# andrewmilson/sandstorm

Hardware: AMD Instinct MI355X
Metric: prove_wall_time_s (lower is better)
Workload: dtype u256 (Fp252, Montgomery R=2^256, 8 x u32 limbs)

## Files before the change

sandstorm_amd/csrc/capi.hip:

```cpp
#include <hip/hip_runtime.h>
#include <dlfcn.h>
#include <algorithm>
#include <cstdarg>
#include <chrono>
#include <cstdio>
#include <cstdlib>
#include <cstring>
#include <map>
#include <mutex>
#include <string>
#include <tuple>
#include <utility>
#include <vector>

#include "../../include/sandstorm_hip.h"
#include "fp252.h"
#include "fp252_host.h"
#include "kernels.h"
#include "quotient_gen.h"
#include "ext_scan.h"
#include "gl_ntt.h"

using namespace ss;

// ... 955 lines not shown
                          const void *d_leaves, uint64_t n, uint8_t *d_nodes, uint8_t *d_tags,
                          uint8_t root_out[33]) {
    return ss_merkle_build_ex(ctx, tree_kind, n_friendly_layers, leaf_kind, d_leaves, n, SS_ORDER_NATURAL, d_nodes, d_tags, root_out);
}
ss_status ss_merkle_build_ex(ss_ctx *ctx, int tree_kind, uint32_t n_friendly_layers, int leaf_kind,
                             const void *d_leaves, uint64_t n, int leaf_order, uint8_t *d_nodes, uint8_t *d_tags,
                             uint8_t root_out[33]) {
    if (!ctx || !d_leaves || !d_nodes) return fail(SS_ERR_INVALID, "NULL argument");
    if (n < 2 || (n & (n - 1))) return fail(SS_ERR_INVALID, "n must be a power of two >= 2");
    if (tree_kind < 0 || tree_kind > SS_TREE_SHA256) return fail(SS_ERR_INVALID, "bad tree kind");
    if (tree_kind == SS_TREE_SHA256 && leaf_kind != SS_LEAF_DIGEST) return fail(SS_ERR_UNSUPPORTED, "SHA-256 trees take digests as leaves");
    if (leaf_kind != SS_LEAF_DIGEST && leaf_kind != SS_LEAF_FELT) return fail(SS_ERR_INVALID, "bad leaf kind %d", leaf_kind);
    if (leaf_order != SS_ORDER_NATURAL && leaf_order != SS_ORDER_BITREV) return fail(SS_ERR_INVALID, "bad leaf order %d", leaf_order);
    uint32_t log_n = 0;
    while ((1ull << log_n) < n) ++log_n;
    if (leaf_kind == SS_LEAF_FELT && leaf_order == SS_ORDER_BITREV) {
        ss_status pst = ctx->ensure_scratch2(n * sizeof(Fp));
        if (pst != SS_OK) return pst;
        HIP_TRY(launch_bitrev_copy(ctx->stream, (const Fp *)d_leaves, log_n, (Fp *)ctx->scratch2));
        d_leaves = ctx->scratch2;
    }
    hipStream_t s = ctx->stream;
    const int hk = tree_kind == SS_TREE_KECCAK ? SS_HASH_KECCAK : tree_kind == SS_TREE_KECCAK_M20 ? SS_HASH_KECCAK_M20
                 : tree_kind == SS_TREE_BLAKE2S ? SS_HASH_BLAKE2S : tree_kind == SS_TREE_SHA256 ? SS_HASH_SHA256 : SS_HASH_BLAKE2S_M20;
    if (tree_kind == SS_TREE_FRIENDLY && !ctx->ped) HIP_TRY(pedersen_tables_create(s, &ctx->ped));
    Fp *ped_tmp = nullptr;
    if (tree_kind == SS_TREE_FRIENDLY) {
        ss_status st = ctx->ensure_scratch(PEDERSEN_TMP_FELTS_PER_HASH * (n / 2) * sizeof(Fp));
        if (st != SS_OK) return st;
        ped_tmp = (Fp *)ctx->scratch;
    }
    HIP_TRY(hipMemsetAsync(d_nodes, 0, 64, s));
    if (d_tags) HIP_TRY(hipMemsetAsync(d_tags, 0, 2 * n, s));
    if (leaf_kind == SS_LEAF_FELT) {
        HIP_TRY(launch_felts_to_be(s, (const Fp *)d_leaves, n, d_nodes + 32 * n));
    } else {
        HIP_TRY(hipMemcpyAsync(d_nodes + 32 * n, d_leaves, 32 * n, hipMemcpyDeviceToDevice, s));
        if (d_tags && tree_kind == SS_TREE_FRIENDLY) HIP_TRY(hipMemsetAsync(d_tags + n, 1, n, s));
    }
    ss_ctx::Scope prof(ctx, SS_PROF_MERKLE);
    for (uint32_t d = log_n; d-- > 0;) {
        const uint64_t count = 1ull << d;
        const uint8_t *in = d_nodes + 32 * (2 * count);
        uint8_t *out = d_nodes + 32 * count;
        const bool leaf_level = d == log_n - 1;
        if (tree_kind == SS_TREE_FRIENDLY) {
            const bool pedersen = leaf_kind == SS_LEAF_FELT || d < n_friendly_layers;
            if (leaf_level && leaf_kind == SS_LEAF_FELT) {
                HIP_TRY(launch_pedersen_felt_pairs(s, ctx->ped, (const Fp *)d_leaves, count, out, ped_tmp));
            } else if (pedersen) {
                HIP_TRY(launch_pedersen_pairs(s, ctx->ped, in, count, out, ped_tmp));
            } else {
                HIP_TRY(launch_hash_pairs(s, SS_HASH_BLAKE2S_M20, in, count, out));
                if (d_tags) HIP_TRY(hipMemsetAsync(d_tags + count, 1, count, s));
            }
        } else if (leaf_level && leaf_kind == SS_LEAF_FELT) {
            HIP_TRY(launch_hash_felt_pairs(s, hk, (const Fp *)d_leaves, count, out));
        } else {
            HIP_TRY(launch_hash_pairs(s, hk, in, count, out));
        }
    }
    if (root_out) {
        HIP_TRY(hipMemcpyAsync(root_out, d_nodes + 32, 32, hipMemcpyDeviceToHost, s));
        root_out[32] = 0;
        if (d_tags) HIP_TRY(hipMemcpyAsync(root_out + 32, d_tags + 1, 1, hipMemcpyDeviceToHost, s));
        HIP_TRY(hipStreamSynchronize(s));
        if (!d_tags && tree_kind == SS_TREE_FRIENDLY)
            root_out[32] = (leaf_kind == SS_LEAF_FELT || n_friendly_layers > 0) ? 0 : 1;
    }
    return SS_OK;
}

// ... 1743 lines not shown
```

sandstorm_amd/csrc/deep.hip:

```cpp
#include <hip/hip_runtime.h>
#include <cstdlib>
#include "fp252.h"
#include "fl252.h"
#include "inv252.h"
#include "kernels.h"

namespace ss {

__device__ __forceinline__ Fp dload(const Fp *p) {
    const uint4 *q = reinterpret_cast<const uint4 *>(p);
    uint4 a = q[0], b = q[1];
    Fp r;
    r.v[0] = a.x; r.v[1] = a.y; r.v[2] = a.z; r.v[3] = a.w;
    r.v[4] = b.x; r.v[5] = b.y; r.v[6] = b.z; r.v[7] = b.w;
    return r;
}
__device__ __forceinline__ void dstore(Fp *p, const Fp &x) {
    uint4 *q = reinterpret_cast<uint4 *>(p);
    q[0] = make_uint4(x.v[0], x.v[1], x.v[2], x.v[3]);
    q[1] = make_uint4(x.v[4], x.v[5], x.v[6], x.v[7]);
}

struct ReduceArgs {
    const Fp *in[MAX_COLS];
// ... 149 lines not shown
    const uint64_t out_len = in_len >> levels;
    uint32_t gx = (uint32_t)((out_len + 127) / 128);
    if (gx > 16384) gx = 16384;
    if (gx == 0) gx = 1;
    const dim3 grid(gx, narrays), block(128);
    const int cn = canonical ? 1 : 0;
    const size_t lds = (size_t)max_points * (36u << levels);
    if (lds > 64 * 1024) return hipErrorInvalidValue;
    if (levels == 4) hipLaunchKernelGGL(ood_fold_kernel<4>, grid, block, lds, st, d_arrays, d_points, out_len, cn);
    else if (levels == 3) hipLaunchKernelGGL(ood_fold_kernel<3>, grid, block, lds, st, d_arrays, d_points, out_len, cn);
    else if (levels == 2) hipLaunchKernelGGL(ood_fold_kernel<2>, grid, block, lds, st, d_arrays, d_points, out_len, cn);
    else hipLaunchKernelGGL(ood_fold_kernel<1>, grid, block, lds, st, d_arrays, d_points, out_len, cn);
    return hipGetLastError();
}

__global__ __launch_bounds__(128) void batch_inverse_kernel(Fp *__restrict__ D, uint64_t nchunks, uint32_t log_chunk,
                                                            Fp offset, Fp w, Fp step, Fp step_inv, Fp z, int r280) {
    const uint64_t c = blockIdx.x * (uint64_t)blockDim.x + threadIdx.x;
    if (c >= nchunks) return;
    const uint64_t CH = 1ull << log_chunk;
    const Fl sl = fl_from_fp(step), sil = fl_from_fp(step_inv), zl = fl_from_fp(z);
    Fl x = fl_from_fp(fp_mul(offset, fp_pow_u64(w, c)));
    Fl run = fl_one();
    for (uint64_t k = 0; k < CH; ++k) {
        dstore(D + c + k * nchunks, fl_pack(run));
        run = fl_mul(fl_sub_c<2, 1>(x, zl), run);
        x = fl_mul(x, sl);
    }
    Fl inv = fl_from_fp(fp_inv_safegcd(fl_to_fp(fl_weak_reduce(run))));
    if (r280) { Fp two24 = fp_zero(); two24.v[0] = 1u << 24; inv = fl_mul(inv, fl_from_fp(fp_to_mont(two24))); }
    for (uint64_t k = CH; k-- > 0;) {
        x = fl_mul(x, sil);
        const Fl pre = fl_from_fp(dload(D + c + k * nchunks));
        dstore(D + c + k * nchunks, fl_to_fp(fl_mul(inv, pre)));
        inv = fl_mul(fl_sub_c<2, 1>(x, zl), inv);
    }
}

static uint32_t batch_inverse_log_chunk(uint32_t log_N) {
    uint32_t log_chunk = log_N > 17 ? log_N - 17 : 0;
    if (log_chunk < 4) log_chunk = log_N < 4 ? log_N : 4;
    if (log_chunk > 7) log_chunk = 7;
    static const char *env = getenv("SS_BATCH_INV_LOG_CHUNK");
    if (env) { const uint32_t v = (uint32_t)atoi(env); if (v >= 1 && v <= 10 && v <= log_N) log_chunk = v; }
    return log_chunk;
}

hipError_t launch_batch_inverse(hipStream_t st, Fp *D, uint32_t log_N, const Fp &offset, const Fp &w,
                                const Fp &w_inv, const Fp &z, bool r280) {
    const uint32_t log_chunk = batch_inverse_log_chunk(log_N);
    const uint64_t nchunks = 1ull << (log_N - log_chunk);
    hipLaunchKernelGGL(batch_inverse_kernel, dim3((uint32_t)((nchunks + 127) / 128)), dim3(128), 0, st, D, nchunks,
                       log_chunk, offset, w, fp_pow_u64(w, nchunks), fp_pow_u64(w_inv, nchunks), z, r280 ? 1 : 0);
    return hipGetLastError();
}

hipError_t launch_batch_inverse_range(hipStream_t st, Fp *D, uint64_t len, const Fp &x0, const Fp &w, const Fp &w_inv,
                                      const Fp &z, bool r280) {
    const uint32_t log_chunk = BATCH_INVERSE_RANGE_LOG_CHUNK;
    const uint64_t nchunks = len >> log_chunk;
    if (nchunks == 0) return hipSuccess;
    hipLaunchKernelGGL(batch_inverse_kernel, dim3((uint32_t)((nchunks + 127) / 128)), dim3(128), 0, st, D, nchunks,
                       log_chunk, x0, w, fp_pow_u64(w, nchunks), fp_pow_u64(w_inv, nchunks), z, r280 ? 1 : 0);
    return hipGetLastError();
}

struct DeepArgs {
    const Fp *trace[MAX_COLS];
    const Fp *comp[4];
    const Fp *D;
    const Fp *Dc;
    const uint32_t *tap_shift;
    const Fp *tap_coef;
    const uint32_t *col_desc;
    const Fp *comp_coef;
    Fp comp_k;
    uint32_t ncoldesc, ncomp, log_stride;
    uint64_t count;
    uint32_t d_bias, d_mask;
// ... 201 lines not shown
```

sandstorm_amd/csrc/hash.hip:

```cpp
#include <hip/hip_runtime.h>
#include <cstring>
#include "fp252.h"
#include "kernels.h"

namespace ss {

__constant__ uint64_t KECCAK_RC[24] = {
    0x0000000000000001ull, 0x0000000000008082ull, 0x800000000000808aull, 0x8000000080008000ull,
    0x000000000000808bull, 0x0000000080000001ull, 0x8000000080008081ull, 0x8000000000008009ull,
    0x000000000000008aull, 0x0000000000000088ull, 0x0000000080008009ull, 0x000000008000000aull,
    0x000000008000808bull, 0x800000000000008bull, 0x8000000000008089ull, 0x8000000000008003ull,
    0x8000000000008002ull, 0x8000000000000080ull, 0x000000000000800aull, 0x800000008000000aull,
    0x8000000080008081ull, 0x8000000000008080ull, 0x0000000080000001ull, 0x8000000080008008ull};

struct K64 { uint32_t lo, hi; };
__device__ __forceinline__ K64 k_split(uint64_t x) { K64 r; r.lo = (uint32_t)x; r.hi = (uint32_t)(x >> 32); return r; }
__device__ __forceinline__ uint64_t k_join(const K64 &x) { return ((uint64_t)x.hi << 32) | x.lo; }
template <int N>
__device__ __forceinline__ K64 k_rotl(const K64 &x) {
    K64 r;
    if (N == 0) { r = x; }
    else if (N == 32) { r.lo = x.hi; r.hi = x.lo; }
    else if (N < 32) {
        r.hi = __builtin_amdgcn_alignbit(x.hi, x.lo, 32 - N);
// ... 2 lines not shown
        r.hi = __builtin_amdgcn_alignbit(x.lo, x.hi, 64 - N);
        r.lo = __builtin_amdgcn_alignbit(x.hi, x.lo, 64 - N);
    }
    return r;
}
__device__ __forceinline__ uint32_t k_xor3(uint32_t a, uint32_t b, uint32_t c) { return __builtin_amdgcn_bitop3_b32(a, b, c, 0x96); }
__device__ __forceinline__ uint32_t k_chi(uint32_t a, uint32_t b, uint32_t c) { return __builtin_amdgcn_bitop3_b32(a, b, c, 0xD2); }
__device__ __forceinline__ K64 k_xor5(const K64 &a, const K64 &b, const K64 &c, const K64 &d, const K64 &e) {
    K64 r; r.lo = k_xor3(k_xor3(a.lo, b.lo, c.lo), d.lo, e.lo); r.hi = k_xor3(k_xor3(a.hi, b.hi, c.hi), d.hi, e.hi); return r;
}
__device__ __forceinline__ K64 k_xor(const K64 &a, const K64 &b) { K64 r; r.lo = a.lo ^ b.lo; r.hi = a.hi ^ b.hi; return r; }
__device__ __forceinline__ K64 k_chi64(const K64 &a, const K64 &b, const K64 &c) { K64 r; r.lo = k_chi(a.lo, b.lo, c.lo); r.hi = k_chi(a.hi, b.hi, c.hi); return r; }
template <int N>
__device__ __forceinline__ K64 k_xrot(const K64 &a, const K64 &d) { return k_rotl<N>(k_xor(a, d)); }

__device__ __forceinline__ void keccak_f1600(uint64_t st[25]) {
    K64 s[25];
#pragma unroll
    for (int i = 0; i < 25; ++i) s[i] = k_split(st[i]);
#pragma unroll 1
    for (int round = 0; round < 24; ++round) {
        const K64 c0 = k_xor5(s[0], s[5], s[10], s[15], s[20]), c1 = k_xor5(s[1], s[6], s[11], s[16], s[21]);
        const K64 c2 = k_xor5(s[2], s[7], s[12], s[17], s[22]), c3 = k_xor5(s[3], s[8], s[13], s[18], s[23]);
        const K64 c4 = k_xor5(s[4], s[9], s[14], s[19], s[24]);
        const K64 d0 = k_xor(c4, k_rotl<1>(c1)), d1 = k_xor(c0, k_rotl<1>(c2)), d2 = k_xor(c1, k_rotl<1>(c3));
        const K64 d3 = k_xor(c2, k_rotl<1>(c4)), d4 = k_xor(c3, k_rotl<1>(c0));
        const K64 b0 = k_xor(s[0], d0);
        const K64 b10 = k_xrot<1>(s[1], d1), b20 = k_xrot<62>(s[2], d2), b5 = k_xrot<28>(s[3], d3);
        const K64 b15 = k_xrot<27>(s[4], d4), b16 = k_xrot<36>(s[5], d0), b1 = k_xrot<44>(s[6], d1);
        const K64 b11 = k_xrot<6>(s[7], d2), b21 = k_xrot<55>(s[8], d3), b6 = k_xrot<20>(s[9], d4);
        const K64 b7 = k_xrot<3>(s[10], d0), b17 = k_xrot<10>(s[11], d1), b2 = k_xrot<43>(s[12], d2);
        const K64 b12 = k_xrot<25>(s[13], d3), b22 = k_xrot<39>(s[14], d4), b23 = k_xrot<41>(s[15], d0);
        const K64 b8 = k_xrot<45>(s[16], d1), b18 = k_xrot<15>(s[17], d2), b3 = k_xrot<21>(s[18], d3);
        const K64 b13 = k_xrot<8>(s[19], d4), b14 = k_xrot<18>(s[20], d0), b24 = k_xrot<2>(s[21], d1);
        const K64 b9 = k_xrot<61>(s[22], d2), b19 = k_xrot<56>(s[23], d3), b4 = k_xrot<14>(s[24], d4);
        s[0] = k_chi64(b0, b1, b2); s[1] = k_chi64(b1, b2, b3); s[2] = k_chi64(b2, b3, b4); s[3] = k_chi64(b3, b4, b0); s[4] = k_chi64(b4, b0, b1);
        s[5] = k_chi64(b5, b6, b7); s[6] = k_chi64(b6, b7, b8); s[7] = k_chi64(b7, b8, b9); s[8] = k_chi64(b8, b9, b5); s[9] = k_chi64(b9, b5, b6);
        s[10] = k_chi64(b10, b11, b12); s[11] = k_chi64(b11, b12, b13); s[12] = k_chi64(b12, b13, b14); s[13] = k_chi64(b13, b14, b10); s[14] = k_chi64(b14, b10, b11);
        s[15] = k_chi64(b15, b16, b17); s[16] = k_chi64(b16, b17, b18); s[17] = k_chi64(b17, b18, b19); s[18] = k_chi64(b18, b19, b15); s[19] = k_chi64(b19, b15, b16);
        s[20] = k_chi64(b20, b21, b22); s[21] = k_chi64(b21, b22, b23); s[22] = k_chi64(b22, b23, b24); s[23] = k_chi64(b23, b24, b20); s[24] = k_chi64(b24, b20, b21);
        const uint64_t rc = KECCAK_RC[round];
        s[0].lo ^= (uint32_t)rc; s[0].hi ^= (uint32_t)(rc >> 32);
    }
#pragma unroll
    for (int i = 0; i < 25; ++i) st[i] = k_join(s[i]);
}

__device__ __forceinline__ uint32_t bswap32(uint32_t x) { return __builtin_bswap32(x); }
__device__ __forceinline__ uint64_t bswap64(uint64_t x) { return __builtin_bswap64(x); }

__device__ __forceinline__ uint64_t felt_msg_lane(const uint64_t *elem, int k) {
    return bswap64(elem[3 - k]);
}

__device__ __forceinline__ void keccak_store_digest(const uint64_t s[25], uint8_t *out, bool mask20) {
    uint64_t o2 = s[2], o3 = s[3];
    if (mask20) { o2 &= 0xffffffffull; o3 = 0; }
    ulonglong2 *q = reinterpret_cast<ulonglong2 *>(out);
    q[0] = make_ulonglong2(s[0], s[1]);
    q[1] = make_ulonglong2(o2, o3);
}

template <typename Fetch>
__device__ __forceinline__ void keccak_absorb_felts(uint64_t s[25], uint32_t nelem, Fetch fetch) {
    const uint32_t data_lanes = 4 * nelem;
    const uint32_t nblocks = data_lanes / 17 + 1;
    for (uint32_t blk = 0; blk < nblocks; ++blk) {
#pragma unroll
        for (int pos = 0; pos < 17; ++pos) {
            const uint32_t lane = blk * 17 + pos;
            if (lane < data_lanes) s[pos] ^= felt_msg_lane(fetch(lane >> 2), lane & 3);
            else if (lane == data_lanes) s[pos] ^= 0x01ull;
        }
        if (blk == nblocks - 1) s[16] ^= 0x8000000000000000ull;
        keccak_f1600(s);
    }
}

__device__ __forceinline__ uint64_t digest_slot(uint64_t row, uint32_t brev_bits) {
    return brev_bits ? (__brevll(row) >> (64u - brev_bits)) : row;
}

__global__ __launch_bounds__(256) void keccak_rows_kernel(ConstColPtrs cols, uint32_t ncols, uint64_t nrows,
                                                          uint8_t *__restrict__ out, int mask20, uint32_t brev_bits) {
    for (uint64_t row = blockIdx.x * (uint64_t)blockDim.x + threadIdx.x; row < nrows;
         row += (uint64_t)gridDim.x * blockDim.x) {
        uint64_t s[25];
#pragma unroll
        for (int i = 0; i < 25; ++i) s[i] = 0;
        keccak_absorb_felts(s, ncols, [&](uint32_t c) {
            return reinterpret_cast<const uint64_t *>(cols.p[c]) + 4 * row;
        });
        keccak_store_digest(s, out + 32 * digest_slot(row, brev_bits), mask20 != 0);
    }
}

__global__ __launch_bounds__(256) void keccak_rows_u64_kernel(ConstColPtrs segs, uint32_t nseg, uint32_t seg_len, uint64_t nrows,
                                                              uint8_t *__restrict__ out) {
    const uint32_t data_lanes = nseg * seg_len, nblocks = data_lanes / 17 + 1;
    for (uint64_t row = blockIdx.x * (uint64_t)blockDim.x + threadIdx.x; row < nrows; row += (uint64_t)gridDim.x * blockDim.x) {
        uint64_t s[25];
#pragma unroll
        for (int i = 0; i < 25; ++i) s[i] = 0;
        uint32_t seg = 0, e = 0;
        for (uint32_t blk = 0; blk < nblocks; ++blk) {
#pragma unroll
            for (int pos = 0; pos < 17; ++pos) {
// ... 8 lines not shown
            }
            if (blk == nblocks - 1) s[16] ^= 0x8000000000000000ull;
            keccak_f1600(s);
        }
        keccak_store_digest(s, out + 32 * row, false);
    }
}
__global__ void gather_rows_u64_kernel(ConstColPtrs segs, uint32_t nseg, uint32_t seg_len, const uint64_t *__restrict__ idx, uint32_t nidx,
                                       uint64_t *__restrict__ out) {
    const uint32_t per = nseg * seg_len, t = blockIdx.x * blockDim.x + threadIdx.x;
    if (t >= nidx * per) return;
    const uint32_t j = t / per, r = t - j * per, s = r / seg_len, e = r - s * seg_len;
    out[t] = reinterpret_cast<const uint64_t *>(segs.p[s])[idx[j] * seg_len + e];
}

__global__ __launch_bounds__(256) void keccak_felt_pairs_kernel(const uint64_t *__restrict__ felts, uint64_t count,
                                                                uint8_t *__restrict__ out, int mask20) {
    for (uint64_t k = blockIdx.x * (uint64_t)blockDim.x + threadIdx.x; k < count;
         k += (uint64_t)gridDim.x * blockDim.x) {
        uint64_t s[25];
#pragma unroll
        for (int i = 0; i < 25; ++i) s[i] = 0;
        keccak_absorb_felts(s, 2, [&](uint32_t c) { return felts + 4 * (2 * k + c); });
        keccak_store_digest(s, out + 32 * k, mask20 != 0);
    }
}

__global__ __launch_bounds__(256) void keccak_pairs_kernel(const uint8_t *__restrict__ in, uint64_t count,
                                                           uint8_t *__restrict__ out, int mask20) {
    for (uint64_t k = blockIdx.x * (uint64_t)blockDim.x + threadIdx.x; k < count;
         k += (uint64_t)gridDim.x * blockDim.x) {
        uint64_t s[25];
        const ulonglong2 *q = reinterpret_cast<const ulonglong2 *>(in + 64 * k);
#pragma unroll
        for (int i = 0; i < 4; ++i) { ulonglong2 v = q[i]; s[2 * i] = v.x; s[2 * i + 1] = v.y; }
        s[8] = 0x01ull;
#pragma unroll
        for (int i = 9; i < 25; ++i) s[i] = 0;
        s[16] = 0x8000000000000000ull;
        keccak_f1600(s);
        keccak_store_digest(s, out + 32 * k, mask20 != 0);
    }
}

__device__ __forceinline__ uint32_t rotr32(uint32_t x, int n) { return __builtin_rotateright32(x, n); }

#define B2S_G(a, b, c, d, x, y)                       \
    a = a + b + (x); d = rotr32(d ^ a, 16);           \
    c = c + d;       b = rotr32(b ^ c, 12);           \
    a = a + b + (y); d = rotr32(d ^ a, 8);            \
    c = c + d;       b = rotr32(b ^ c, 7);

#define B2S_ROUND(s0, s1, s2, s3, s4, s5, s6, s7, s8, s9, s10, s11, s12, s13, s14, s15) \
    B2S_G(v0, v4, v8, v12, m[s0], m[s1]);   B2S_G(v1, v5, v9, v13, m[s2], m[s3]);       \
    B2S_G(v2, v6, v10, v14, m[s4], m[s5]);  B2S_G(v3, v7, v11, v15, m[s6], m[s7]);      \
// ... 62 lines not shown
    }
}

__global__ __launch_bounds__(256) void blake2s_rows_kernel(ConstColPtrs cols, uint32_t ncols, uint64_t nrows,
                                                           uint8_t *__restrict__ out, int mask20, uint32_t brev_bits) {
    for (uint64_t row = blockIdx.x * (uint64_t)blockDim.x + threadIdx.x; row < nrows;
         row += (uint64_t)gridDim.x * blockDim.x) {
        uint32_t h[8];
        blake2s_hash_felts(h, ncols, [&](uint32_t c) {
            return load_fp(reinterpret_cast<const uint8_t *>(cols.p[c]) + 32 * row);
        });
        blake2s_store_digest(h, out + 32 * digest_slot(row, brev_bits), mask20 != 0);
    }
}

__global__ __launch_bounds__(256) void blake2s_felt_pairs_kernel(const Fp *__restrict__ felts, uint64_t count,
                                                                 uint8_t *__restrict__ out, int mask20) {
    for (uint64_t k = blockIdx.x * (uint64_t)blockDim.x + threadIdx.x; k < count;
         k += (uint64_t)gridDim.x * blockDim.x) {
        uint32_t h[8];
        blake2s_hash_felts(h, 2, [&](uint32_t c) { return load_fp(felts + 2 * k + c); });
        blake2s_store_digest(h, out + 32 * k, mask20 != 0);
    }
}

__global__ __launch_bounds__(256) void blake2s_pairs_kernel(const uint8_t *__restrict__ in, uint64_t count,
                                                            uint8_t *__restrict__ out, int mask20) {
    for (uint64_t k = blockIdx.x * (uint64_t)blockDim.x + threadIdx.x; k < count;
         k += (uint64_t)gridDim.x * blockDim.x) {
        uint32_t h[8], m[16];
        const uint4 *q = reinterpret_cast<const uint4 *>(in + 64 * k);
#pragma unroll
        for (int i = 0; i < 4; ++i) { uint4 v = q[i]; m[4 * i] = v.x; m[4 * i + 1] = v.y; m[4 * i + 2] = v.z; m[4 * i + 3] = v.w; }
        blake2s_init(h);
        blake2s_compress(h, m, 64, true);
        blake2s_store_digest(h, out + 32 * k, mask20 != 0);
    }
}

__global__ __launch_bounds__(256) void felts_to_be_kernel(const Fp *__restrict__ felts, uint64_t count,
                                                          uint8_t *__restrict__ out) {
    for (uint64_t k = blockIdx.x * (uint64_t)blockDim.x + threadIdx.x; k < count;
         k += (uint64_t)gridDim.x * blockDim.x) {
        Fp e = load_fp(felts + k);
        uint4 *q = reinterpret_cast<uint4 *>(out + 32 * k);
        q[0] = make_uint4(bswap32(e.v[7]), bswap32(e.v[6]), bswap32(e.v[5]), bswap32(e.v[4]));
        q[1] = make_uint4(bswap32(e.v[3]), bswap32(e.v[2]), bswap32(e.v[1]), bswap32(e.v[0]));
    }
}

struct Digest32 { uint64_t w[4]; };

__global__ void pow_prefix_kernel(int coin_kind, Digest32 digest, uint32_t bits, uint64_t *__restrict__ prefix) {
    if (threadIdx.x != 0 || blockIdx.x != 0) return;
    const uint64_t magic = 0x0123456789ABCDEDull;
    if (coin_kind == 0) {
        uint64_t s[25];
#pragma unroll
        for (int k = 0; k < 25; ++k) s[k] = 0;
        s[0] = bswap64(magic);
        s[1] = digest.w[0]; s[2] = digest.w[1]; s[3] = digest.w[2]; s[4] = digest.w[3];
        s[5] = (uint64_t)(bits & 0xffu) | (0x01ull << 8);
        s[16] = 0x8000000000000000ull;
// ... 190 lines not shown
    if (kind == 0) hipLaunchKernelGGL(keccak_rows_u64_kernel, dim3(grid_for(nrows, 256, 1u << 20)), dim3(256), 0, st, segs, nseg, seg_len, nrows, digests);
    else if (kind == 2) hipLaunchKernelGGL(sha256_rows_u64_kernel, dim3(grid_for(nrows, 256, 1u << 20)), dim3(256), 0, st, segs, nseg, seg_len, nrows, digests);
    else hipLaunchKernelGGL(blake2s_rows_u64_kernel, dim3(grid_for(nrows, 256, 1u << 20)), dim3(256), 0, st, segs, nseg, seg_len, nrows, digests);
    return hipGetLastError();
}
hipError_t launch_gather_rows_u64(hipStream_t st, const ConstColPtrs &segs, uint32_t nseg, uint32_t seg_len, const uint64_t *d_idx, uint32_t nidx,
                                  uint64_t *d_out) {
    const uint32_t total = nidx * nseg * seg_len;
    if (!total) return hipSuccess;
    hipLaunchKernelGGL(gather_rows_u64_kernel, dim3((total + 255) / 256), dim3(256), 0, st, segs, nseg, seg_len, d_idx, nidx, d_out);
    return hipGetLastError();
}
hipError_t launch_hash_rows(hipStream_t st, int kind, const ConstColPtrs &cols, uint32_t ncols,
                            uint64_t nrows, uint32_t brev_bits, uint8_t *digests) {
    const uint32_t grid = grid_for(nrows, 256, 1u << 20);
    if (kind == 0 || kind == 1)
        hipLaunchKernelGGL(keccak_rows_kernel, dim3(grid), dim3(256), 0, st, cols, ncols, nrows, digests, kind == 1, brev_bits);
    else
        hipLaunchKernelGGL(blake2s_rows_kernel, dim3(grid), dim3(256), 0, st, cols, ncols, nrows, digests, kind == 3, brev_bits);
    return hipGetLastError();
}
__global__ __launch_bounds__(256) void bitrev_copy_kernel(const Fp *__restrict__ src, uint32_t log_n, Fp *__restrict__ dst) {
    const uint64_t n = 1ull << log_n;
    for (uint64_t i = blockIdx.x * (uint64_t)blockDim.x + threadIdx.x; i < n; i += (uint64_t)gridDim.x * blockDim.x) {
        const uint64_t j = log_n ? (__brevll(i) >> (64u - log_n)) : 0;
        const uint4 *q = reinterpret_cast<const uint4 *>(src + j);
        uint4 *d = reinterpret_cast<uint4 *>(dst + i);
        d[0] = q[0]; d[1] = q[1];
    }
}
hipError_t launch_bitrev_copy(hipStream_t st, const Fp *src, uint32_t log_n, Fp *dst) {
    hipLaunchKernelGGL(bitrev_copy_kernel, dim3(grid_for(1ull << log_n, 256, 1u << 20)), dim3(256), 0, st, src, log_n, dst);
    return hipGetLastError();
}
hipError_t launch_hash_pairs(hipStream_t st, int kind, const uint8_t *in, uint64_t count, uint8_t *out) {
    const uint32_t grid = grid_for(count, 256, 1u << 20);
    if (kind == 4)
        hipLaunchKernelGGL(sha256_pairs_kernel, dim3(grid), dim3(256), 0, st, in, count, out);
    else if (kind == 0 || kind == 1)
        hipLaunchKernelGGL(keccak_pairs_kernel, dim3(grid), dim3(256), 0, st, in, count, out, kind == 1);
    else
        hipLaunchKernelGGL(blake2s_pairs_kernel, dim3(grid), dim3(256), 0, st, in, count, out, kind == 3);
    return hipGetLastError();
}
hipError_t launch_hash_felt_pairs(hipStream_t st, int kind, const Fp *felts, uint64_t count, uint8_t *out) {
    const uint32_t grid = grid_for(count, 256, 1u << 20);
    if (kind == 0 || kind == 1)
        hipLaunchKernelGGL(keccak_felt_pairs_kernel, dim3(grid), dim3(256), 0, st,
                           reinterpret_cast<const uint64_t *>(felts), count, out, kind == 1);
    else
        hipLaunchKernelGGL(blake2s_felt_pairs_kernel, dim3(grid), dim3(256), 0, st, felts, count, out, kind == 3);
    return hipGetLastError();
}
hipError_t launch_felts_to_be(hipStream_t st, const Fp *felts, uint64_t count, uint8_t *out) {
    hipLaunchKernelGGL(felts_to_be_kernel, dim3(grid_for(count, 256, 1u << 20)), dim3(256), 0, st, felts, count, out);
    return hipGetLastError();
}
hipError_t launch_pow_prefix(hipStream_t st, int coin_kind, const uint8_t digest[32], uint32_t bits,
                             uint64_t *d_prefix) {
    Digest32 d;
    memcpy(d.w, digest, 32);
    hipLaunchKernelGGL(pow_prefix_kernel, dim3(1), dim3(64), 0, st, coin_kind, d, bits, d_prefix);
    return hipGetLastError();
}
hipError_t launch_pow_grind(hipStream_t st, int coin_kind, const uint64_t *d_prefix, uint32_t bits,
                            uint64_t start, uint64_t count, unsigned long long *d_best) {
// ... 25 lines not shown
```

sandstorm_amd/csrc/kernels.h:

```cpp
#pragma once
#include <hip/hip_runtime.h>
#include <stdint.h>
#include "fp252.h"

namespace ss {

static constexpr int MAX_COLS = 16;

struct ColPtrs {
    const void *src[MAX_COLS];
    void *dst[MAX_COLS];
};
struct ConstColPtrs {
    const void *p[MAX_COLS];
};

int ntt_log_tile_max();
static constexpr size_t NTT_PLAN_ENTRY_BYTES = 36;
enum { NTT_MODE_DIT = 0, NTT_MODE_DIF = 1, NTT_MODE_CTI = 2 };
struct NttWindow { uint32_t first, log_len; };
hipError_t launch_ntt_pass(hipStream_t st, int mode, const ColPtrs &cols, uint32_t ncols, const Fp *tw,
                           uint32_t log_n, uint32_t s0, uint32_t r, uint32_t log_tile, uint32_t u_first,
                           uint32_t log_expand, uint32_t scale_pow2, bool final_pass, bool cti_trivial = true,
                           const NttWindow *win = nullptr, uint64_t tw_entries = 0);
hipError_t launch_twiddles(hipStream_t st, Fp *tw, const Fp *pow_lo, const Fp *pow_hi, const Fp *hpow,
                           uint32_t log_n, bool h_is_one, bool bitrev_levels, const NttWindow *win = nullptr, uint32_t win_stages = 0);
static inline uint64_t ntt_window_plan_entries(const NttWindow &win, uint32_t stages) { return (((uint64_t)1 << stages) - 1ull) << win.log_len; }
hipError_t launch_bitrev(hipStream_t st, Fp *a, uint32_t log_n);
hipError_t launch_mul_bench(hipStream_t st, const Fp *a, const Fp *b, Fp *out, uint64_t n, uint32_t reps);
hipError_t ntt_set_func_attributes();

hipError_t launch_hash_rows(hipStream_t st, int kind, const ConstColPtrs &cols, uint32_t ncols,
                            uint64_t nrows, uint32_t brev_bits, uint8_t *digests);
hipError_t launch_bitrev_copy(hipStream_t st, const Fp *src, uint32_t log_n, Fp *dst);
hipError_t launch_hash_pairs(hipStream_t st, int kind, const uint8_t *in, uint64_t count, uint8_t *out);
hipError_t launch_hash_felt_pairs(hipStream_t st, int kind, const Fp *felts, uint64_t count, uint8_t *out);
hipError_t launch_felts_to_be(hipStream_t st, const Fp *felts, uint64_t count, uint8_t *out);
hipError_t launch_pow_prefix(hipStream_t st, int coin_kind, const uint8_t digest[32], uint32_t bits,
                             uint64_t *d_prefix);
hipError_t launch_pow_grind(hipStream_t st, int coin_kind, const uint64_t *d_prefix, uint32_t bits,
                            uint64_t start, uint64_t count, unsigned long long *d_best);
hipError_t launch_gather32(hipStream_t st, const uint8_t *in, const uint64_t *d_idx, uint64_t n, uint8_t *out);
hipError_t launch_gather32_cols(hipStream_t st, const void *const *d_cols, uint32_t ncols, uint32_t c0, uint32_t row_cols, const uint64_t *d_idx,
                                uint64_t nidx, uint8_t *out);
hipError_t launch_gather8(hipStream_t st, const uint8_t *in, const uint64_t *d_idx, uint64_t n, uint8_t *out);

struct PedersenTables;
hipError_t pedersen_tables_create(hipStream_t st, PedersenTables **out);
void pedersen_tables_destroy(PedersenTables *t);
void pedersen_tables_trim();
static constexpr uint64_t PEDERSEN_TMP_FELTS_PER_HASH = 4;
// ... 170 lines not shown
```

Measured before the change: 0.2198.

## Add descent batch inverse, fused bitrev felt-pair hashing, specialized Keccak rows and squeeze

Batch inversion gains a recursive descent scheme that inverts a smaller squared domain and expands it four ways per level. It also adds a zero-aware fallback pass, gated by a device flag, for when a denominator vanishes. Merkle leaf hashing for felt leaves now reads bit-reversed input directly and writes big-endian leaves inside the hash kernel, which removes the separate bitrev copy and felts_to_be passes. Keccak gets column-count-specialized row kernels and a truncated final round that computes only the four output lanes. These changes add extra kernel launches and a global flag ring, and enlarge the set of template instantiations.

```diff
diff --git a/sandstorm_amd/csrc/capi.hip b/sandstorm_amd/csrc/capi.hip
--- a/sandstorm_amd/csrc/capi.hip
+++ b/sandstorm_amd/csrc/capi.hip
@@ -993,7 +993,8 @@
     if (leaf_order != SS_ORDER_NATURAL && leaf_order != SS_ORDER_BITREV) return fail(SS_ERR_INVALID, "bad leaf order %d", leaf_order);
     uint32_t log_n = 0;
     while ((1ull << log_n) < n) ++log_n;
-    if (leaf_kind == SS_LEAF_FELT && leaf_order == SS_ORDER_BITREV) {
+    const bool leaves_bitrev = leaf_kind == SS_LEAF_FELT && leaf_order == SS_ORDER_BITREV && tree_kind != SS_TREE_FRIENDLY;
+    if (leaf_kind == SS_LEAF_FELT && leaf_order == SS_ORDER_BITREV && !leaves_bitrev) {
         ss_status pst = ctx->ensure_scratch2(n * sizeof(Fp));
         if (pst != SS_OK) return pst;
         HIP_TRY(launch_bitrev_copy(ctx->stream, (const Fp *)d_leaves, log_n, (Fp *)ctx->scratch2));
@@ -1012,7 +1013,7 @@
     HIP_TRY(hipMemsetAsync(d_nodes, 0, 64, s));
     if (d_tags) HIP_TRY(hipMemsetAsync(d_tags, 0, 2 * n, s));
     if (leaf_kind == SS_LEAF_FELT) {
-        HIP_TRY(launch_felts_to_be(s, (const Fp *)d_leaves, n, d_nodes + 32 * n));
+        if (tree_kind == SS_TREE_FRIENDLY) HIP_TRY(launch_felts_to_be(s, (const Fp *)d_leaves, n, d_nodes + 32 * n));
     } else {
         HIP_TRY(hipMemcpyAsync(d_nodes + 32 * n, d_leaves, 32 * n, hipMemcpyDeviceToDevice, s));
         if (d_tags && tree_kind == SS_TREE_FRIENDLY) HIP_TRY(hipMemsetAsync(d_tags + n, 1, n, s));
@@ -1034,7 +1035,7 @@
                 if (d_tags) HIP_TRY(hipMemsetAsync(d_tags + count, 1, count, s));
             }
         } else if (leaf_level && leaf_kind == SS_LEAF_FELT) {
-            HIP_TRY(launch_hash_felt_pairs(s, hk, (const Fp *)d_leaves, count, out));
+            HIP_TRY(launch_hash_felt_pairs(s, hk, (const Fp *)d_leaves, count, leaves_bitrev, out, d_nodes + 32 * n));
         } else {
             HIP_TRY(launch_hash_pairs(s, hk, in, count, out));
         }
diff --git a/sandstorm_amd/csrc/deep.hip b/sandstorm_amd/csrc/deep.hip
--- a/sandstorm_amd/csrc/deep.hip
+++ b/sandstorm_amd/csrc/deep.hip
@@ -1,5 +1,7 @@
 #include <hip/hip_runtime.h>
+#include <atomic>
 #include <cstdlib>
+#include <mutex>
 #include "fp252.h"
 #include "fl252.h"
 #include "inv252.h"
@@ -187,26 +189,36 @@
     return hipGetLastError();
 }
 
+template <bool ZERO_AWARE>
 __global__ __launch_bounds__(128) void batch_inverse_kernel(Fp *__restrict__ D, uint64_t nchunks, uint32_t log_chunk,
-                                                            Fp offset, Fp w, Fp step, Fp step_inv, Fp z, int r280) {
+                                                            Fp offset, Fp w, Fp step, Fp step_inv, Fp z, int r280,
+                                                            uint32_t *__restrict__ flag, uint32_t ticket) {
     const uint64_t c = blockIdx.x * (uint64_t)blockDim.x + threadIdx.x;
     if (c >= nchunks) return;
+    if (ZERO_AWARE && *flag != ticket) return;
     const uint64_t CH = 1ull << log_chunk;
     const Fl sl = fl_from_fp(step), sil = fl_from_fp(step_inv), zl = fl_from_fp(z);
     Fl x = fl_from_fp(fp_mul(offset, fp_pow_u64(w, c)));
     Fl run = fl_one();
     for (uint64_t k = 0; k < CH; ++k) {
         dstore(D + c + k * nchunks, fl_pack(run));
-        run = fl_mul(fl_sub_c<2, 1>(x, zl), run);
+        Fl d = fl_sub_c<2, 1>(x, zl);
+        if (ZERO_AWARE) { d = fl_weak_reduce(d); if (fn_is_zero(d)) d = fl_one(); }
+        run = fl_mul(d, run);
         x = fl_mul(x, sl);
     }
-    Fl inv = fl_from_fp(fp_inv_safegcd(fl_to_fp(fl_weak_reduce(run))));
+    const Fp inv_fp = fp_inv_safegcd(fl_to_fp(fl_weak_reduce(run)));
+    if (!ZERO_AWARE && flag && fp_is_zero(inv_fp)) *flag = ticket;
+    Fl inv = fl_from_fp(inv_fp);
     if (r280) { Fp two24 = fp_zero(); two24.v[0] = 1u << 24; inv = fl_mul(inv, fl_from_fp(fp_to_mont(two24))); }
     for (uint64_t k = CH; k-- > 0;) {
         x = fl_mul(x, sil);
         const Fl pre = fl_from_fp(dload(D + c + k * nchunks));
-        dstore(D + c + k * nchunks, fl_to_fp(fl_mul(inv, pre)));
-        inv = fl_mul(fl_sub_c<2, 1>(x, zl), inv);
+        Fl d = fl_sub_c<2, 1>(x, zl);
+        bool zero = false;
+        if (ZERO_AWARE) { d = fl_weak_reduce(d); zero = fn_is_zero(d); if (zero) d = fl_one(); }
+        dstore(D + c + k * nchunks, zero ? fp_zero() : fl_to_fp(fl_mul(inv, pre)));
+        inv = fl_mul(d, inv);
     }
 }
 
@@ -219,13 +231,103 @@
     return log_chunk;
 }
 
+static hipError_t launch_batch_inverse_strided(hipStream_t st, Fp *D, uint64_t nchunks, uint32_t log_chunk, const Fp &x0, const Fp &w, const Fp &w_inv,
+                                               const Fp &z, bool r280, uint32_t *flag, uint32_t ticket, bool zero_aware) {
+    const dim3 grid((uint32_t)((nchunks + 127) / 128)), block(128);
+    const Fp step = fp_pow_u64(w, nchunks), step_inv = fp_pow_u64(w_inv, nchunks);
+    if (zero_aware) hipLaunchKernelGGL(batch_inverse_kernel<true>, grid, block, 0, st, D, nchunks, log_chunk, x0, w, step, step_inv, z, r280 ? 1 : 0, flag, ticket);
+    else hipLaunchKernelGGL(batch_inverse_kernel<false>, grid, block, 0, st, D, nchunks, log_chunk, x0, w, step, step_inv, z, r280 ? 1 : 0, flag, ticket);
+    return hipGetLastError();
+}
+static hipError_t launch_batch_inverse_chunks(hipStream_t st, Fp *D, uint32_t log_N, const Fp &offset, const Fp &w, const Fp &w_inv,
+                                              const Fp &z, bool r280, uint32_t *flag, uint32_t ticket, bool zero_aware) {
+    return launch_batch_inverse_strided(st, D, 1ull << (log_N - batch_inverse_log_chunk(log_N)), batch_inverse_log_chunk(log_N), offset, w, w_inv, z,
+                                        r280, flag, ticket, zero_aware);
+}
+
+__global__ __launch_bounds__(128) void inverse_descent_kernel(Fp *__restrict__ D, uint64_t q, uint64_t lanes, Fp a, Fp g, Fp step, Fp t, Fp c,
+                                                              Fp c2, int final, const uint32_t *__restrict__ flag, uint32_t ticket) {
+    const uint64_t l = blockIdx.x * (uint64_t)blockDim.x + threadIdx.x;
+    if (l >= lanes || *flag == ticket) return;
+    const Fl sl = fl_from_fp(step), tl = fl_from_fp(t), cl = fl_from_fp(c), c2l = fl_from_fp(c2);
+    Fl y = fl_from_fp(a), gp = fl_from_fp(g);
+    for (uint64_t b = l; b; b >>= 1) {
+        if (b & 1) y = fl_mul(y, gp);
+        gp = fl_sqr(gp);
+    }
+    Fp e_next = dload(D + l);
+    for (uint64_t i = l; i < q; i += lanes) {
+        const Fl e = fl_from_fp(e_next);
+        if (i + lanes < q) e_next = dload(D + i + lanes);
+        const Fl y2 = fl_sqr(y), ty = fl_mul(y, tl);
+        const Fl f0 = fl_mul(fl_add(y2, c2l), e), f1 = fl_mul(fl_sub_c<2, 1>(c2l, y2), e);
+        const Fl r0 = fl_mul(fl_add(y, cl), f0), r2 = fl_mul(fl_sub_c<2, 1>(cl, y), f0);
+        const Fl r1 = fl_mul(fl_add(ty, cl), f1), r3 = fl_mul(fl_sub_c<2, 1>(cl, ty), f1);
+        if (final) {
+            dstore(D + i, fl_to_fp(r0)); dstore(D + i + q, fl_to_fp(r1)); dstore(D + i + 2 * q, fl_to_fp(r2)); dstore(D + i + 3 * q, fl_to_fp(r3));
+        } else {
+            dstore(D + i, fl_pack(r0)); dstore(D + i + q, fl_pack(r1)); dstore(D + i + 2 * q, fl_pack(r2)); dstore(D + i + 3 * q, fl_pack(r3));
+        }
+        y = fl_mul(y, sl);
+    }
+}
+
+static constexpr uint32_t BATCH_INVERSE_DESCENT_LAST_LOG = 19, BATCH_INVERSE_DESCENT_LANES = 3 * 64 * 1024;
+static uint32_t batch_inverse_descent_last_log() {
+    if (const char *e = getenv("SS_BATCH_INV_DESCENT_LAST_LOG")) { const uint32_t v = (uint32_t)atoi(e); if (v >= 4 && v <= 40) return v; }
+    return BATCH_INVERSE_DESCENT_LAST_LOG;
+}
+
+static constexpr uint32_t DESCENT_FLAG_SLOTS = 1024, DESCENT_MAX_DEVICES = 64;
+static hipError_t descent_flag(uint32_t **flag, uint32_t *ticket) {
+    static std::mutex mu;
+    static uint32_t *ring[DESCENT_MAX_DEVICES] = {};
+    static std::atomic<uint32_t> next{0};
+    int dev = 0;
+    hipError_t e = hipGetDevice(&dev);
+    if (e != hipSuccess) return e;
+    if (dev < 0 || dev >= (int)DESCENT_MAX_DEVICES) return hipErrorInvalidDevice;
+    {
+        std::lock_guard<std::mutex> lock(mu);
+        if (!ring[dev]) {
+            uint32_t *p = nullptr;
+            if ((e = hipMalloc((void **)&p, DESCENT_FLAG_SLOTS * sizeof(uint32_t))) != hipSuccess) return e;
+            static const uint32_t zeros[DESCENT_FLAG_SLOTS] = {};
+            if ((e = hipMemcpy(p, zeros, sizeof zeros, hipMemcpyHostToDevice)) != hipSuccess) { (void)hipFree(p); return e; }
+            ring[dev] = p;
+        }
+    }
+    uint32_t k = next.fetch_add(1u) + 1u;
+    if (k == 0) k = next.fetch_add(1u) + 1u;
+    *ticket = k;
+    *flag = ring[dev] + k % DESCENT_FLAG_SLOTS;
+    return hipSuccess;
+}
+
 hipError_t launch_batch_inverse(hipStream_t st, Fp *D, uint32_t log_N, const Fp &offset, const Fp &w,
                                 const Fp &w_inv, const Fp &z, bool r280) {
-    const uint32_t log_chunk = batch_inverse_log_chunk(log_N);
-    const uint64_t nchunks = 1ull << (log_N - log_chunk);
-    hipLaunchKernelGGL(batch_inverse_kernel, dim3((uint32_t)((nchunks + 127) / 128)), dim3(128), 0, st, D, nchunks,
-                       log_chunk, offset, w, fp_pow_u64(w, nchunks), fp_pow_u64(w_inv, nchunks), z, r280 ? 1 : 0);
-    return hipGetLastError();
+    uint32_t *flag = nullptr, ticket = 0;
+    hipError_t e = descent_flag(&flag, &ticket);
+    if (e != hipSuccess) return e;
+    const uint32_t last_log = batch_inverse_descent_last_log();
+    if (log_N < last_log + 3) {
+        if ((e = launch_batch_inverse_chunks(st, D, log_N, offset, w, w_inv, z, r280, flag, ticket, false)) != hipSuccess) return e;
+        return launch_batch_inverse_chunks(st, D, log_N, offset, w, w_inv, z, r280, flag, ticket, true);
+    }
+    const uint32_t J = (log_N - last_log) & ~1u;
+    Fp a[64], g[64], gi[64], c[64];
+    a[0] = offset; g[0] = w; gi[0] = w_inv; c[0] = z;
+    for (uint32_t j = 1; j <= J; ++j) { a[j] = fp_sqr(a[j - 1]); g[j] = fp_sqr(g[j - 1]); gi[j] = fp_sqr(gi[j - 1]); c[j] = fp_sqr(c[j - 1]); }
+    if ((e = launch_batch_inverse_chunks(st, D, log_N - J, a[J], g[J], gi[J], c[J], r280, flag, ticket, false)) != hipSuccess) return e;
+    for (uint32_t j = J; j >= 2; j -= 2) {
+        const uint32_t lv = j - 2;
+        const uint64_t q = 1ull << (log_N - j);
+        const uint64_t lanes = q < BATCH_INVERSE_DESCENT_LANES ? q : BATCH_INVERSE_DESCENT_LANES;
+        hipLaunchKernelGGL(inverse_descent_kernel, dim3((uint32_t)((lanes + 127) / 128)), dim3(128), 0, st, D, q, lanes, a[lv], g[lv],
+                           fp_pow_u64(g[lv], lanes), fp_pow_u64(g[lv], q), c[lv], c[lv + 1], lv == 0 ? 1 : 0, flag, ticket);
+        if ((e = hipGetLastError()) != hipSuccess) return e;
+    }
+    return launch_batch_inverse_chunks(st, D, log_N, offset, w, w_inv, z, r280, flag, ticket, true);
 }
 
 hipError_t launch_batch_inverse_range(hipStream_t st, Fp *D, uint64_t len, const Fp &x0, const Fp &w, const Fp &w_inv,
@@ -233,9 +335,11 @@
     const uint32_t log_chunk = BATCH_INVERSE_RANGE_LOG_CHUNK;
     const uint64_t nchunks = len >> log_chunk;
     if (nchunks == 0) return hipSuccess;
-    hipLaunchKernelGGL(batch_inverse_kernel, dim3((uint32_t)((nchunks + 127) / 128)), dim3(128), 0, st, D, nchunks,
-                       log_chunk, x0, w, fp_pow_u64(w, nchunks), fp_pow_u64(w_inv, nchunks), z, r280 ? 1 : 0);
-    return hipGetLastError();
+    uint32_t *flag = nullptr, ticket = 0;
+    hipError_t e = descent_flag(&flag, &ticket);
+    if (e != hipSuccess) return e;
+    if ((e = launch_batch_inverse_strided(st, D, nchunks, log_chunk, x0, w, w_inv, z, r280, flag, ticket, false)) != hipSuccess) return e;
+    return launch_batch_inverse_strided(st, D, nchunks, log_chunk, x0, w, w_inv, z, r280, flag, ticket, true);
 }
 
 struct DeepArgs {
diff --git a/sandstorm_amd/csrc/hash.hip b/sandstorm_amd/csrc/hash.hip
--- a/sandstorm_amd/csrc/hash.hip
+++ b/sandstorm_amd/csrc/hash.hip
@@ -40,17 +40,17 @@
 template <int N>
 __device__ __forceinline__ K64 k_xrot(const K64 &a, const K64 &d) { return k_rotl<N>(k_xor(a, d)); }
 
-__device__ __forceinline__ void keccak_f1600(uint64_t st[25]) {
-    K64 s[25];
-#pragma unroll
-    for (int i = 0; i < 25; ++i) s[i] = k_split(st[i]);
+#define KECCAK_THETA(s)                                                                                                 \
+    const K64 c0 = k_xor5(s[0], s[5], s[10], s[15], s[20]), c1 = k_xor5(s[1], s[6], s[11], s[16], s[21]);               \
+    const K64 c2 = k_xor5(s[2], s[7], s[12], s[17], s[22]), c3 = k_xor5(s[3], s[8], s[13], s[18], s[23]);               \
+    const K64 c4 = k_xor5(s[4], s[9], s[14], s[19], s[24]);                                                             \
+    const K64 d0 = k_xor(c4, k_rotl<1>(c1)), d1 = k_xor(c0, k_rotl<1>(c2)), d2 = k_xor(c1, k_rotl<1>(c3));              \
+    const K64 d3 = k_xor(c2, k_rotl<1>(c4)), d4 = k_xor(c3, k_rotl<1>(c0));
+
+__device__ __forceinline__ void keccak_rounds(K64 (&s)[25], int nrounds) {
 #pragma unroll 1
-    for (int round = 0; round < 24; ++round) {
-        const K64 c0 = k_xor5(s[0], s[5], s[10], s[15], s[20]), c1 = k_xor5(s[1], s[6], s[11], s[16], s[21]);
-        const K64 c2 = k_xor5(s[2], s[7], s[12], s[17], s[22]), c3 = k_xor5(s[3], s[8], s[13], s[18], s[23]);
-        const K64 c4 = k_xor5(s[4], s[9], s[14], s[19], s[24]);
-        const K64 d0 = k_xor(c4, k_rotl<1>(c1)), d1 = k_xor(c0, k_rotl<1>(c2)), d2 = k_xor(c1, k_rotl<1>(c3));
-        const K64 d3 = k_xor(c2, k_rotl<1>(c4)), d4 = k_xor(c3, k_rotl<1>(c0));
+    for (int round = 0; round < nrounds; ++round) {
+        KECCAK_THETA(s)
         const K64 b0 = k_xor(s[0], d0);
         const K64 b10 = k_xrot<1>(s[1], d1), b20 = k_xrot<62>(s[2], d2), b5 = k_xrot<28>(s[3], d3);
         const K64 b15 = k_xrot<27>(s[4], d4), b16 = k_xrot<36>(s[5], d0), b1 = k_xrot<44>(s[6], d1);
@@ -68,8 +68,32 @@
         const uint64_t rc = KECCAK_RC[round];
         s[0].lo ^= (uint32_t)rc; s[0].hi ^= (uint32_t)(rc >> 32);
     }
+}
+
+__device__ __forceinline__ void keccak_f1600(uint64_t st[25]) {
+    K64 s[25];
+#pragma unroll
+    for (int i = 0; i < 25; ++i) s[i] = k_split(st[i]);
+    keccak_rounds(s, 24);
 #pragma unroll
     for (int i = 0; i < 25; ++i) st[i] = k_join(s[i]);
+}
+
+__device__ __forceinline__ void keccak_f1600_squeeze4(uint64_t st[25]) {
+    K64 s[25];
+#pragma unroll
+    for (int i = 0; i < 25; ++i) s[i] = k_split(st[i]);
+    keccak_rounds(s, 23);
+    {
+        KECCAK_THETA(s)
+        const K64 b0 = k_xor(s[0], d0), b1 = k_xrot<44>(s[6], d1), b2 = k_xrot<43>(s[12], d2);
+        const K64 b3 = k_xrot<21>(s[18], d3), b4 = k_xrot<14>(s[24], d4);
+        s[0] = k_chi64(b0, b1, b2); s[1] = k_chi64(b1, b2, b3); s[2] = k_chi64(b2, b3, b4); s[3] = k_chi64(b3, b4, b0);
+        const uint64_t rc = 0x8000000080008008ull;
+        s[0].lo ^= (uint32_t)rc; s[0].hi ^= (uint32_t)(rc >> 32);
+    }
+#pragma unroll
+    for (int i = 0; i < 4; ++i) st[i] = k_join(s[i]);
 }
 
 __device__ __forceinline__ uint32_t bswap32(uint32_t x) { return __builtin_bswap32(x); }
@@ -91,16 +115,64 @@
 __device__ __forceinline__ void keccak_absorb_felts(uint64_t s[25], uint32_t nelem, Fetch fetch) {
     const uint32_t data_lanes = 4 * nelem;
     const uint32_t nblocks = data_lanes / 17 + 1;
-    for (uint32_t blk = 0; blk < nblocks; ++blk) {
+    auto absorb = [&](uint32_t blk) {
 #pragma unroll
         for (int pos = 0; pos < 17; ++pos) {
             const uint32_t lane = blk * 17 + pos;
             if (lane < data_lanes) s[pos] ^= felt_msg_lane(fetch(lane >> 2), lane & 3);
             else if (lane == data_lanes) s[pos] ^= 0x01ull;
         }
-        if (blk == nblocks - 1) s[16] ^= 0x8000000000000000ull;
+    };
+    for (uint32_t blk = 0; blk + 1 < nblocks; ++blk) {
+        absorb(blk);
         keccak_f1600(s);
     }
+    absorb(nblocks - 1);
+    s[16] ^= 0x8000000000000000ull;
+    keccak_f1600_squeeze4(s);
+}
+
+template <int NC, int BLK>
+__device__ __forceinline__ void keccak_absorb_block(uint64_t s[25], const uint64_t (&m)[4 * NC]) {
+    constexpr int DL = 4 * NC, NB = DL / 17 + 1;
+    if constexpr (BLK < NB) {
+#pragma unroll
+        for (int pos = 0; pos < 17; ++pos) {
+            constexpr int base = BLK * 17;
+            if (base + pos < DL) s[pos] ^= m[base + pos < DL ? base + pos : 0];
+            else if (base + pos == DL) s[pos] ^= 0x01ull;
+        }
+        if constexpr (BLK == NB - 1) {
+            s[16] ^= 0x8000000000000000ull;
+            keccak_f1600_squeeze4(s);
+        } else {
+            keccak_f1600(s);
+        }
+        keccak_absorb_block<NC, BLK + 1>(s, m);
+    }
+}
+template <int NC>
+__device__ __forceinline__ void keccak_load_felts(uint64_t (&m)[4 * NC], const uint4 *const (&e)[NC]) {
+#pragma unroll
+    for (int c = 0; c < NC; ++c) {
+        const uint4 a = e[c][0], b = e[c][1];
+        m[4 * c + 0] = bswap64(((uint64_t)b.w << 32) | b.z);
+        m[4 * c + 1] = bswap64(((uint64_t)b.y << 32) | b.x);
+        m[4 * c + 2] = bswap64(((uint64_t)a.w << 32) | a.z);
+        m[4 * c + 3] = bswap64(((uint64_t)a.y << 32) | a.x);
+    }
+}
+template <int NC>
+__device__ __forceinline__ void keccak_hash_lanes(uint64_t s[25], const uint64_t (&m)[4 * NC]) {
+#pragma unroll
+    for (int i = 0; i < 25; ++i) s[i] = 0;
+    keccak_absorb_block<NC, 0>(s, m);
+}
+template <int NC>
+__device__ __forceinline__ void keccak_hash_felts(uint64_t s[25], const uint4 *const (&e)[NC]) {
+    uint64_t m[4 * NC];
+    keccak_load_felts<NC>(m, e);
+    keccak_hash_lanes<NC>(s, m);
 }
 
 __device__ __forceinline__ uint64_t digest_slot(uint64_t row, uint32_t brev_bits) {
@@ -117,6 +189,23 @@
         keccak_absorb_felts(s, ncols, [&](uint32_t c) {
             return reinterpret_cast<const uint64_t *>(cols.p[c]) + 4 * row;
         });
+        keccak_store_digest(s, out + 32 * digest_slot(row, brev_bits), mask20 != 0);
+    }
+}
+
+template <int NC>
+__global__ __launch_bounds__(256) void keccak_rows_w_kernel(ConstColPtrs cols, uint64_t nrows, uint8_t *__restrict__ out, int mask20,
+                                                            uint32_t brev_bits) {
+    const uint4 *col[NC];
+#pragma unroll
+    for (int c = 0; c < NC; ++c) col[c] = reinterpret_cast<const uint4 *>(cols.p[c]);
+    for (uint64_t row = blockIdx.x * (uint64_t)blockDim.x + threadIdx.x; row < nrows;
+         row += (uint64_t)gridDim.x * blockDim.x) {
+        const uint4 *e[NC];
+#pragma unroll
+        for (int c = 0; c < NC; ++c) e[c] = col[c] + 2 * row;
+        uint64_t s[25];
+        keccak_hash_felts<NC>(s, e);
         keccak_store_digest(s, out + 32 * digest_slot(row, brev_bits), mask20 != 0);
     }
 }
@@ -155,15 +244,21 @@
     out[t] = reinterpret_cast<const uint64_t *>(segs.p[s])[idx[j] * seg_len + e];
 }
 
-__global__ __launch_bounds__(256) void keccak_felt_pairs_kernel(const uint64_t *__restrict__ felts, uint64_t count,
-                                                                uint8_t *__restrict__ out, int mask20) {
+__global__ __launch_bounds__(256) void keccak_felt_pairs_kernel(const uint4 *__restrict__ felts, uint64_t count, uint8_t *__restrict__ out,
+                                                                uint8_t *__restrict__ leaves, int mask20, uint32_t brev_bits) {
     for (uint64_t k = blockIdx.x * (uint64_t)blockDim.x + threadIdx.x; k < count;
          k += (uint64_t)gridDim.x * blockDim.x) {
-        uint64_t s[25];
-#pragma unroll
-        for (int i = 0; i < 25; ++i) s[i] = 0;
-        keccak_absorb_felts(s, 2, [&](uint32_t c) { return felts + 4 * (2 * k + c); });
-        keccak_store_digest(s, out + 32 * k, mask20 != 0);
+        const uint4 *e[2] = {felts + 2 * (brev_bits ? k : 2 * k), felts + 2 * (brev_bits ? k + count : 2 * k + 1)};
+        const uint64_t slot = digest_slot(k, brev_bits);
+        uint64_t s[25], m[8];
+        keccak_load_felts<2>(m, e);
+        if (leaves) {
+            ulonglong2 *q = reinterpret_cast<ulonglong2 *>(leaves + 64 * slot);
+#pragma unroll
+            for (int i = 0; i < 4; ++i) q[i] = make_ulonglong2(m[2 * i], m[2 * i + 1]);
+        }
+        keccak_hash_lanes<2>(s, m);
+        keccak_store_digest(s, out + 32 * slot, mask20 != 0);
     }
 }
 
@@ -179,7 +274,7 @@
 #pragma unroll
         for (int i = 9; i < 25; ++i) s[i] = 0;
         s[16] = 0x8000000000000000ull;
-        keccak_f1600(s);
+        keccak_f1600_squeeze4(s);
         keccak_store_digest(s, out + 32 * k, mask20 != 0);
     }
 }
@@ -272,13 +367,21 @@
     }
 }
 
-__global__ __launch_bounds__(256) void blake2s_felt_pairs_kernel(const Fp *__restrict__ felts, uint64_t count,
-                                                                 uint8_t *__restrict__ out, int mask20) {
+__device__ __forceinline__ void store_felt_be(const Fp &e, uint8_t *out) {
+    uint4 *q = reinterpret_cast<uint4 *>(out);
+    q[0] = make_uint4(bswap32(e.v[7]), bswap32(e.v[6]), bswap32(e.v[5]), bswap32(e.v[4]));
+    q[1] = make_uint4(bswap32(e.v[3]), bswap32(e.v[2]), bswap32(e.v[1]), bswap32(e.v[0]));
+}
+__global__ __launch_bounds__(256) void blake2s_felt_pairs_kernel(const Fp *__restrict__ felts, uint64_t count, uint8_t *__restrict__ out,
+                                                                 uint8_t *__restrict__ leaves, int mask20, uint32_t brev_bits) {
     for (uint64_t k = blockIdx.x * (uint64_t)blockDim.x + threadIdx.x; k < count;
          k += (uint64_t)gridDim.x * blockDim.x) {
+        const Fp e0 = load_fp(brev_bits ? felts + k : felts + 2 * k), e1 = load_fp(brev_bits ? felts + k + count : felts + 2 * k + 1);
+        const uint64_t slot = digest_slot(k, brev_bits);
+        if (leaves) { store_felt_be(e0, leaves + 64 * slot); store_felt_be(e1, leaves + 64 * slot + 32); }
         uint32_t h[8];
-        blake2s_hash_felts(h, 2, [&](uint32_t c) { return load_fp(felts + 2 * k + c); });
-        blake2s_store_digest(h, out + 32 * k, mask20 != 0);
+        blake2s_hash_felts(h, 2, [&](uint32_t c) { return c ? e1 : e0; });
+        blake2s_store_digest(h, out + 32 * slot, mask20 != 0);
     }
 }
 
@@ -299,12 +402,8 @@
 __global__ __launch_bounds__(256) void felts_to_be_kernel(const Fp *__restrict__ felts, uint64_t count,
                                                           uint8_t *__restrict__ out) {
     for (uint64_t k = blockIdx.x * (uint64_t)blockDim.x + threadIdx.x; k < count;
-         k += (uint64_t)gridDim.x * blockDim.x) {
-        Fp e = load_fp(felts + k);
-        uint4 *q = reinterpret_cast<uint4 *>(out + 32 * k);
-        q[0] = make_uint4(bswap32(e.v[7]), bswap32(e.v[6]), bswap32(e.v[5]), bswap32(e.v[4]));
-        q[1] = make_uint4(bswap32(e.v[3]), bswap32(e.v[2]), bswap32(e.v[1]), bswap32(e.v[0]));
-    }
+         k += (uint64_t)gridDim.x * blockDim.x)
+        store_felt_be(load_fp(felts + k), out + 32 * k);
 }
 
 struct Digest32 { uint64_t w[4]; };
@@ -525,9 +624,15 @@
 hipError_t launch_hash_rows(hipStream_t st, int kind, const ConstColPtrs &cols, uint32_t ncols,
                             uint64_t nrows, uint32_t brev_bits, uint8_t *digests) {
     const uint32_t grid = grid_for(nrows, 256, 1u << 20);
-    if (kind == 0 || kind == 1)
-        hipLaunchKernelGGL(keccak_rows_kernel, dim3(grid), dim3(256), 0, st, cols, ncols, nrows, digests, kind == 1, brev_bits);
-    else
+    if (kind == 0 || kind == 1) {
+        const int m20 = kind == 1;
+        switch (ncols) {
+#define SS_KECCAK_ROWS_W(NC) case NC: hipLaunchKernelGGL(keccak_rows_w_kernel<NC>, dim3(grid), dim3(256), 0, st, cols, nrows, digests, m20, brev_bits); break;
+            SS_KECCAK_ROWS_W(1) SS_KECCAK_ROWS_W(2) SS_KECCAK_ROWS_W(4) SS_KECCAK_ROWS_W(7) SS_KECCAK_ROWS_W(8) SS_KECCAK_ROWS_W(9) SS_KECCAK_ROWS_W(10)
+#undef SS_KECCAK_ROWS_W
+            default: hipLaunchKernelGGL(keccak_rows_kernel, dim3(grid), dim3(256), 0, st, cols, ncols, nrows, digests, m20, brev_bits);
+        }
+    } else
         hipLaunchKernelGGL(blake2s_rows_kernel, dim3(grid), dim3(256), 0, st, cols, ncols, nrows, digests, kind == 3, brev_bits);
     return hipGetLastError();
 }
@@ -554,13 +659,19 @@
         hipLaunchKernelGGL(blake2s_pairs_kernel, dim3(grid), dim3(256), 0, st, in, count, out, kind == 3);
     return hipGetLastError();
 }
-hipError_t launch_hash_felt_pairs(hipStream_t st, int kind, const Fp *felts, uint64_t count, uint8_t *out) {
-    const uint32_t grid = grid_for(count, 256, 1u << 20);
+static inline uint32_t log2_exact(uint64_t n) {
+    uint32_t l = 0;
+    while ((1ull << l) < n) ++l;
+    return l;
+}
+hipError_t launch_hash_felt_pairs(hipStream_t st, int kind, const Fp *felts, uint64_t count, bool bitrev, uint8_t *out, uint8_t *leaves) {
+    if (bitrev && (count & (count - 1))) return hipErrorInvalidValue;
+    const uint32_t grid = grid_for(count, 256, 1u << 20), brev_bits = bitrev ? log2_exact(count) : 0;
     if (kind == 0 || kind == 1)
         hipLaunchKernelGGL(keccak_felt_pairs_kernel, dim3(grid), dim3(256), 0, st,
-                           reinterpret_cast<const uint64_t *>(felts), count, out, kind == 1);
+                           reinterpret_cast<const uint4 *>(felts), count, out, leaves, kind == 1, brev_bits);
     else
-        hipLaunchKernelGGL(blake2s_felt_pairs_kernel, dim3(grid), dim3(256), 0, st, felts, count, out, kind == 3);
+        hipLaunchKernelGGL(blake2s_felt_pairs_kernel, dim3(grid), dim3(256), 0, st, felts, count, out, leaves, kind == 3, brev_bits);
     return hipGetLastError();
 }
 hipError_t launch_felts_to_be(hipStream_t st, const Fp *felts, uint64_t count, uint8_t *out) {
diff --git a/sandstorm_amd/csrc/kernels.h b/sandstorm_amd/csrc/kernels.h
--- a/sandstorm_amd/csrc/kernels.h
+++ b/sandstorm_amd/csrc/kernels.h
@@ -34,7 +34,7 @@
                             uint64_t nrows, uint32_t brev_bits, uint8_t *digests);
 hipError_t launch_bitrev_copy(hipStream_t st, const Fp *src, uint32_t log_n, Fp *dst);
 hipError_t launch_hash_pairs(hipStream_t st, int kind, const uint8_t *in, uint64_t count, uint8_t *out);
-hipError_t launch_hash_felt_pairs(hipStream_t st, int kind, const Fp *felts, uint64_t count, uint8_t *out);
+hipError_t launch_hash_felt_pairs(hipStream_t st, int kind, const Fp *felts, uint64_t count, bool bitrev, uint8_t *out, uint8_t *leaves);
 hipError_t launch_felts_to_be(hipStream_t st, const Fp *felts, uint64_t count, uint8_t *out);
 hipError_t launch_pow_prefix(hipStream_t st, int coin_kind, const uint8_t digest[32], uint32_t bits,
                              uint64_t *d_prefix);
```

Measured after the change: 0.2168 (median of 6 runs). -1.4%, faster.
